# SAIC-MONTREAL/multimodal-dynamics

Measured on AMD Instinct MI355X. Metric: visuotactile samples/sec (train) + ELBO vs CPU ref, cnn-mvae 64x64 bs256 @1/2/4/8 GPU, higher is better.
Workload: dtype f32x3; 1 GPU; cnn-mvae visuotactile+pose 64x64, bs=256 per GPU, fp32 storage and results, GEMMs in the fp32x3 arithmetic (exact three-term bf16 split of the fp32 operands, six of nine products on the bf16 matrix cores, fp32 accumulate; error vs fp64 <= native fp32 MFMA), seq_modeling train step (7 subset ELBOs + backward + Adam), BASELINE configs[1]; global_batch=256, parallelism=dp1, bn=local, launch=hip_graph

## Files before the change

include/mmdyn_hip.h:

```cpp
#ifndef MMDYN_HIP_H
#define MMDYN_HIP_H

#include <stdint.h>

#ifdef __cplusplus
extern "C" {
#endif

#define MMDYN_OK 0
#define MMDYN_ERR_SHAPE (-1)
#define MMDYN_ERR_NULL (-2)
#define MMDYN_ERR_RANGE (-3)

#define MMDYN_ACT_NONE 0
#define MMDYN_ACT_SWISH 1
#define MMDYN_ACT_RELU 2

#define MMDYN_DENSE 0
#define MMDYN_CONV 1
#define MMDYN_TCONV_S2P1 2
#define MMDYN_IM2COL3 3

#define MMDYN_TCONV_S1P0 4

// ... 333 lines not shown
                      int Wi, int Cg, int stride, int offset, int chunks, int flags, void* stream);
int mmdyn_split_planes(const float* x, void* planes, int64_t rows, int C, void* stream);
int mmdyn_igemm_planes_served(int mode, int G, int Bg, int Hi, int Wi, int Cin, int Ho, int Wo, int N);
int mmdyn_bn_swish_fwd_planes(const float* y, const float* mean, const float* rstd, const float* gamma, const float* beta,
                              float* a, void* a_planes, int G, int rows_per_group, int C, void* stream);
int mmdyn_bn_swish_bwd_apply_planes(const float* da, const float* y, const float* mean, const float* rstd, const float* gamma,
                                    const float* beta, const float* sums, float* dy, void* dy_planes, int G, int rows_per_group,
                                    int C, int da_is_du, void* stream);
int mmdyn_conv3_fwd_planes(const float* x, const float* Wp, float* C, void* act_planes, int G, int Bg, int H, int act,
                           void* stream);
int mmdyn_conv3_dgrad_bn_stats(const float* dlogits, const float* Wp, float* stats, const float* y, const float* mean,
                               const float* rstd, const float* gamma, const float* beta, int G, int Bg, int H, void* stream);
int mmdyn_conv3_dgrad_bn_apply_planes(const float* dlogits, const float* Wp, const float* y, const float* mean,
                                      const float* rstd, const float* gamma, const float* beta, const float* sums,
                                      void* dy_planes, int G, int Bg, int H, void* stream);
int mmdyn_bn_eval_swish_bwd(const float* da, const float* y, const float* mean, const float* rstd, const float* gamma,
                            const float* beta, float* dy, void* dy_planes, float* partial, int G, int rows_per_group, int C,
                            int da_is_du, void* stream);
int mmdyn_bn_swish_fwd_b16(const uint16_t* y, const float* mean, const float* rstd, const float* gamma,
                           const float* beta, uint16_t* a, int G, int rows_per_group, int C, int half, void* stream);
int mmdyn_bn_swish_bwd_reduce_b16(const uint16_t* da, const uint16_t* y, const float* mean, const float* rstd,
                                  const float* gamma, const float* beta, float* partial, int G, int rows_per_group,
                                  int C, int half, void* stream);
int mmdyn_bn_swish_bwd_apply_b16(const uint16_t* da, const uint16_t* y, const float* mean, const float* rstd,
                                 const float* gamma, const float* beta, const float* sums, uint16_t* dy, int G,
                                 int rows_per_group, int C, int da_is_du, int half, void* stream);
int mmdyn_act_bwd_b16(const uint16_t* dh, const uint16_t* u, uint16_t* du, int64_t n, int act, int half, void* stream);
int mmdyn_tconv_out3_fwd_b16(const uint16_t* a, const float* w, float* out, int Bt, int Hi, int Wi, int half,
                             void* stream);

// ... 13 lines not shown
```

multimodal-dynamics_amd/csrc/bn.hip:

```cpp
#include "common.h"

namespace {

static int tile_rows_for(int rows_per_group) {
  int t = rows_per_group / 256 / 32 * 32;
  return t < 32 ? 32 : (t > 512 ? 512 : t);
}

struct BnParams {
  const float* mean;
  const float* rstd;
  const float* gamma;
  const float* beta;
};

template <int MODE, typename TA>
__global__ __launch_bounds__(256) void colreduce_kernel(const TA* __restrict__ y,
                                                        const TA* __restrict__ da, BnParams bp,
                                                        float* __restrict__ partial, int rows_per_group,
                                                        int C, int T, int tile_rows) {
  __shared__ float red[256 * 8];
  const int tid = threadIdx.x;
  const int g = blockIdx.y, t = blockIdx.x;
  const int CV = C >> 2;
// ... 301 lines not shown
  for (int64_t i = blockIdx.x * (int64_t)blockDim.x + threadIdx.x; i < total8; i += (int64_t)gridDim.x * blockDim.x) {
    const int cv = (int)(i % CV);
    const int64_t row = i / CV;
    const int g = (int)(row / rows_per_group);
    f32x4 v[2], o[2];
    ldv_nt<float>(y + i * 8, v);
    ldv_nt<float>(y + i * 8 + 4, v + 1);
#pragma unroll
    for (int q = 0; q < 2; ++q) {
      const int c0 = cv * 8 + q * 4;
      f32x4 m = *reinterpret_cast<const f32x4*>(bp.mean + (size_t)g * C + c0);
      f32x4 r = *reinterpret_cast<const f32x4*>(bp.rstd + (size_t)g * C + c0);
      f32x4 ga = *reinterpret_cast<const f32x4*>(bp.gamma + c0);
      f32x4 be = *reinterpret_cast<const f32x4*>(bp.beta + c0);
#pragma unroll
      for (int k = 0; k < 4; ++k) o[q][k] = swishf_(ga[k] * ((v[q][k] - m[k]) * r[k]) + be[k]);
    }
    if (a) {
      stv_nt<float>(a + i * 8, o);
      stv_nt<float>(a + i * 8 + 4, o + 1);
    }
    store_planes8(ap + row * 3 * (int64_t)C + cv * 8, C, o[0], o[1]);
  }
}

__global__ void bn_swish_bwd_apply_planes_kernel(const float* __restrict__ da, const float* __restrict__ y, BnParams bp,
                                                 const float* __restrict__ sums, float* __restrict__ dy, bf16_t* __restrict__ dyp,
                                                 int64_t total8, int rows_per_group, int C, int da_is_du) {
  const int CV = C / 8;
  const float inv_n = 1.f / (float)rows_per_group;
  for (int64_t i = blockIdx.x * (int64_t)blockDim.x + threadIdx.x; i < total8; i += (int64_t)gridDim.x * blockDim.x) {
// ... 367 lines not shown
```

multimodal-dynamics_amd/csrc/common.h:

```cpp
#pragma once
#include <hip/hip_runtime.h>
#include <stdint.h>
#include <stdlib.h>
#include "mmdyn_hip.h"

typedef float f32x16 __attribute__((ext_vector_type(16)));
typedef float f32x4 __attribute__((ext_vector_type(4)));

typedef uint16_t bf16_t;
template <typename T> __device__ __forceinline__ f32x4 ld4(const T* p);
template <> __device__ __forceinline__ f32x4 ld4<float>(const float* p) { return *reinterpret_cast<const f32x4*>(p); }
template <> __device__ __forceinline__ f32x4 ld4<bf16_t>(const bf16_t* p) {
  const uint2 u = *reinterpret_cast<const uint2*>(p);
  f32x4 v;
  v[0] = __uint_as_float(u.x << 16);
  v[1] = __uint_as_float(u.x & 0xffff0000u);
  v[2] = __uint_as_float(u.y << 16);
  v[3] = __uint_as_float(u.y & 0xffff0000u);
  return v;
}
template <typename T> __device__ __forceinline__ float ld1(const T* p);
template <> __device__ __forceinline__ float ld1<float>(const float* p) { return *p; }
template <> __device__ __forceinline__ float ld1<bf16_t>(const bf16_t* p) { return __uint_as_float((uint32_t)*p << 16); }
__device__ __forceinline__ uint32_t pack2_bf16(float lo, float hi) {
// ... 232 lines not shown
  v = wave_sum_d(v);
  __shared__ double red[4];
  if ((threadIdx.x & 63) == 0) red[threadIdx.x >> 6] = v;
  __syncthreads();
  if (threadIdx.x == 0) atomicAdd(dst, scale * (red[0] + red[1] + red[2] + red[3]));
}

constexpr float POE_EPS = 1e-8f;

constexpr uint32_t ALL_PRESENT = 0x01010101u;
__device__ __forceinline__ bool has(uint32_t word, int m) { return ((word >> (8 * m)) & 0xffu) != 0u; }

__device__ __forceinline__ float sigmoid_exact(float v) { return 1.f / (1.f + expf(-v)); }
__device__ __forceinline__ float sigmoidf_(float x) { return __builtin_amdgcn_rcpf(1.0f + __expf(-x)); }
__device__ __forceinline__ float swishf_(float x) { return x * sigmoidf_(x); }
__device__ __forceinline__ float swish_gradf_(float x) {
  float s = sigmoidf_(x);
  return s * (1.0f + x * (1.0f - s));
}
__device__ __forceinline__ float bn_swish_bwd_dy(float du, float xh, float ga, float r, float s0, float s1, float inv_n,
                                                 bool tail_fused) {
#pragma clang fp contract(off)
  const float t0 = __builtin_fmaf(-inv_n, s0, du);
  const float s1n = inv_n * s1;
  const float t = tail_fused ? __builtin_fmaf(-s1n, xh, t0) : t0 - s1n * xh;
  return (ga * r) * t;
}
__device__ __forceinline__ float apply_act(float x, int act) {
  if (act == MMDYN_ACT_SWISH) return swishf_(x);
  if (act == MMDYN_ACT_RELU) return x > 0.f ? x : 0.f;
// ... 45 lines not shown
```

multimodal-dynamics_amd/csrc/tconv_patch.hip:

```cpp
#include "igemm_geom.h"

namespace {

struct PatchEpi {
  const float* bias;
  float* C_act;
  int act;
  const float* bn_y;
  const float* bn_mean;
  const float* bn_rstd;
  const float* bn_gamma;
  const float* bn_beta;
  int bwd_act;
};

typedef __bf16 bf16x8v __attribute__((ext_vector_type(8)));

template <int H, int W, int CIN, int N, int TH, bool P3>
struct PatchCfg {
  static constexpr int CP = CIN + 4, PW2 = W + 2, PH2 = TH + 2;
  static constexpr int ROWB = P3 ? 6 * CIN : 4 * CIN;
  static constexpr int PSB = P3 ? 6 * CIN + 32 : 4 * CP;
  static constexpr int PPP = ROWB / 16;
  static constexpr int NT = N / 16, MT = TH * W / 16 / 8;
  static constexpr int TILES = H / TH;
  static constexpr int SLICE_V = N * PPP;
  static constexpr int NWL = (SLICE_V + 511) / 512;
  static constexpr size_t SMEM = (size_t)(PH2 * PW2 + 2 * N) * PSB;
  static_assert(H % TH == 0 && (TH * W) % 128 == 0 && (W & (W - 1)) == 0 && W >= 16 && CIN % 32 == 0 && N % 16 == 0, "tile geometry");
  static_assert(!P3 || (PSB / 32) % 2 == 1, "plane rows: a stride of 32 * odd bytes");
  static_assert(SMEM <= 160 * 1024, "LDS of one CU");
};

template <int H, int W, int CIN, int N, int TH, bool P3, bool BWD>
__global__ __launch_bounds__(512) void tconv_patch_kernel(const void* __restrict__ X, const void* __restrict__ Wp,
                                                          float* __restrict__ Y, float* __restrict__ stats, int Bt, int Bg,
                                                          int ldc, const PatchEpi ep) {
  using K = PatchCfg<H, W, CIN, N, TH, P3>;
  constexpr int PW2 = K::PW2, PH2 = K::PH2, NT = K::NT, MT = K::MT, PSB = K::PSB, PPP = K::PPP, ROWB = K::ROWB, NWL = K::NWL;
  extern __shared__ __attribute__((aligned(16))) char smem[];
  char* patch = smem;
  char* Bs = smem + PH2 * PW2 * PSB;
  const char* Xb = static_cast<const char*>(X);
  const char* Wb = static_cast<const char*>(Wp);
  const int tid = threadIdx.x, lane = tid & 63, wave = tid >> 6;
  const int r = lane & 15, q = lane >> 4;
  auto widx = [](int s) {
    const int ph = s >> 3, pw = (s >> 2) & 1, th = (s >> 1) & 1, tw = s & 1;
    return (1 - ph + 2 * th) * 4 + (1 - pw + 2 * tw);
  };
  constexpr int RD = 4;
  u32x4_t rb[RD][NWL];
  auto bload = [&](int s, u32x4_t (&dst)[NWL]) {
#pragma unroll
// ... 4 lines not shown
  };
  auto bstore = [&](int slot, const u32x4_t (&src)[NWL]) {
#pragma unroll
    for (int k = 0; k < NWL; ++k) {
      const int i = tid + 512 * k, n = i / PPP, c = i - n * PPP;
      if (i < K::SLICE_V) *reinterpret_cast<u32x4_t*>(Bs + ((size_t)slot * N + n) * PSB + c * 16) = src[k];
    }
  };
  int py_[MT], px_[MT];
#pragma unroll
  for (int m = 0; m < MT; ++m) {
    const int p = (wave * MT + m) * 16 + r;
    py_[m] = p / W;
    px_[m] = p % W;
  }
  constexpr int NPIECE = PH2 * PW2 * PPP, NLD = (NPIECE + 511) / 512;
  const int total = Bt * K::TILES;
  u32x4_t pv[NLD];
  unsigned pok = 0;
  auto pload = [&](int u, int k0, int k1) {
    const int b = u / K::TILES, y0 = (u - b * K::TILES) * TH;
    int t = tid;
    asm volatile("" : "+v"(t));
#pragma unroll
    for (int k = 0; k < NLD; ++k) {
      if (k < k0 || k >= k1) continue;
      const int i = t + 512 * k;
      const int c = i % PPP, p = i / PPP;
      const int py = p / PW2, px = p - py * PW2;
      const int iy = y0 + py - 1, ix = px - 1;
      const bool ok = i < NPIECE && iy >= 0 && iy < H && ix >= 0 && ix < W;
      pok = (pok & ~(1u << k)) | (ok ? 1u << k : 0u);
      pv[k] = __builtin_nontemporal_load(
          reinterpret_cast<const u32x4_t*>(Xb + (ok ? (((size_t)b * H + iy) * W + ix) * ROWB + c * 16 : (size_t)0)));
    }
  };
  auto pstore = [&](int k0, int k1) {
    const u32x4_t z = {0u, 0u, 0u, 0u};
    int t = tid;
    asm volatile("" : "+v"(t));
#pragma unroll
    for (int k = 0; k < NLD; ++k) {
      if (k < k0 || k >= k1) continue;
      const int i = t + 512 * k;
      if (i < NPIECE) *reinterpret_cast<u32x4_t*>(patch + (size_t)(i / PPP) * PSB + (i % PPP) * 16) = ((pok >> k) & 1u) ? pv[k] : z;
    }
  };
  constexpr int NPRE = BWD ? NLD / 2 : NLD, NH = NLD;
  if ((int)blockIdx.x < total) {
    pload(blockIdx.x, 0, NPRE);
#pragma unroll
    for (int k = 0; k < RD; ++k) bload(k, rb[k]);
  }
  for (int u = blockIdx.x; u < total; u += gridDim.x) {
    const int b = u / K::TILES, y0 = (u - b * K::TILES) * TH;
    pload(u, NPRE, NH);
    __syncthreads();
    pstore(0, NH);
    bstore(0, rb[0]);
    __syncthreads();
    if (u + (int)gridDim.x < total) pload(u + gridDim.x, 0, NPRE);
    float colsum[NT], colsq[NT];
#pragma unroll
    for (int n = 0; n < NT; ++n) colsum[n] = colsq[n] = 0.f;
    const int grp_b = b / Bg;
    constexpr bool bnbwd = BWD;
    float bn_m[NT], bn_r[NT], bn_g[NT], bn_b[NT], bias_v[NT];
#pragma unroll
    for (int n = 0; n < NT; ++n) {
      const int col = n * 16 + r;
      const bool bn = bnbwd && ep.bn_mean != nullptr;
      bn_m[n] = bn ? ep.bn_mean[(size_t)grp_b * N + col] : 0.f;
      bn_r[n] = bn ? ep.bn_rstd[(size_t)grp_b * N + col] : 1.f;
      bn_g[n] = bn ? ep.bn_gamma[col] : 1.f;
      bn_b[n] = bn ? ep.bn_beta[col] : 0.f;
      bias_v[n] = ep.bias ? ep.bias[col] : 0.f;
// ... 9 lines not shown
      if constexpr (bnbwd) {
#pragma unroll
        for (int m = 0; m < MT; ++m)
#pragma unroll
          for (int e = 0; e < 4; ++e) {
            const int p = (wave * MT + m) * 16 + 4 * q + e;
            const int y = y0 + p / W, x = p % W;
            const size_t ooff = ((((size_t)b * 2 * H + (2 * y + ph)) * 2 * W) + (2 * x + pw)) * ldc + r;
#pragma unroll
            for (int n = 0; n < NT; ++n) yv[m][e][n] = ep.bn_y[ooff + n * 16];
          }
      }
#pragma unroll
      for (int tap = 0; tap < 4; ++tap) {
        const int s = cls * 4 + tap, slot = tap & 1;
        if (s + 1 < 16) bstore(slot ^ 1, rb[(tap + 1) % RD]);
        bload((s + RD) & 15, rb[tap % RD]);
        const int dh = ph - (tap >> 1), dw = pw - (tap & 1);
        if constexpr (P3) {
          const char* bbase = Bs + ((size_t)slot * N + r) * PSB + q * 16;
          const char* abase[MT];
#pragma unroll
          for (int m = 0; m < MT; ++m) abase[m] = patch + ((size_t)(py_[m] + dh + 1) * PW2 + (px_[m] + dw + 1)) * PSB + q * 16;
          constexpr int order[6][2] = {{0, 2}, {2, 0}, {1, 1}, {0, 1}, {1, 0}, {0, 0}};
#pragma unroll
          for (int kk = 0; kk < CIN / 32; ++kk) {
            bf16x8v bf[NT][3];
#pragma unroll
            for (int n = 0; n < NT; ++n)
#pragma unroll
// ... 99 lines not shown
  if (Hi == 32 && Cin == 32) return 2;
  if (Hi == 64 && Cin == 32) return 8;
  return 0;
}

template <int H, int W, int CIN, int N, int TH, bool P3>
int patch_launch(const void* A, const void* Bp, float* C, float* stats, const IgemmGeom& g, const PatchEpi& ep, hipStream_t st) {
  using K = PatchCfg<H, W, CIN, N, TH, P3>;
  static LdsOptIn lds_opt_in;
  static LdsOptIn lds_opt_in_bwd;
  const int Bt = g.G * g.Bg;
  const int grid = Bt * K::TILES < device_cus() ? Bt * K::TILES : device_cus();
  if (ep.bn_y) {
    if (int e = lds_opt_in_bwd.ensure((const void*)tconv_patch_kernel<H, W, CIN, N, TH, P3, true>, (int)K::SMEM)) return e;
    hipLaunchKernelGGL((tconv_patch_kernel<H, W, CIN, N, TH, P3, true>), dim3(grid), dim3(512), K::SMEM, st, A, Bp, C, stats, Bt, g.Bg,
                       g.ldc, ep);
  } else {
    if (int e = lds_opt_in.ensure((const void*)tconv_patch_kernel<H, W, CIN, N, TH, P3, false>, (int)K::SMEM)) return e;
    hipLaunchKernelGGL((tconv_patch_kernel<H, W, CIN, N, TH, P3, false>), dim3(grid), dim3(512), K::SMEM, st, A, Bp, C, stats, Bt, g.Bg,
                       g.ldc, ep);
  }
  MMDYN_LAUNCH_CHECK();
}

template <bool P3>
int patch_go(const void* A, const void* Bp, const float* bias, float* C, float* C_act, float* stats, float* ws, const IgemmGeom& g,
             hipStream_t st) {
  if (ws || g.splitk != 1) return MMDYN_ERR_SHAPE;
  if (g.bn_y && g.ldc != g.N) return MMDYN_ERR_SHAPE;
  const PatchEpi ep{bias, C_act, g.act, g.bn_y, g.bn_mean, g.bn_rstd, g.bn_gamma, g.bn_beta, g.bwd_act};
  if (g.Hi == 16) return patch_launch<16, 16, 64, 32, 16, P3>(A, Bp, C, stats, g, ep, st);
  if (g.Hi == 32) return patch_launch<32, 32, 32, 32, 16, P3>(A, Bp, C, stats, g, ep, st);
  return patch_launch<64, 64, 32, 32, 8, P3>(A, Bp, C, stats, g, ep, st);
}

// ... 10 lines not shown
bool mmdyn_tconv_patch_plan(const IgemmGeom& g, bool planes, IgemmPlan* p) {
  if (planes && !(patch_p3_enabled() && g.G > 0 && g.Bg > 0)) return false;
  const int tiles = patch_tiles(g.mode, g.Hi, g.Wi, g.Cin, g.Ho, g.Wo, g.N);
  if (!tiles) return false;
  *p = IgemmPlan{};
  p->family = IGEMM_PATCH;
  p->planes = planes;
  p->stat_tiles = g.Bg * tiles;
  return true;
}

int mmdyn_tconv_patch_launch(const void* A, const void* Bp, const float* bias, float* C, float* C_act, float* stats, float* ws,
                             const IgemmGeom& g, const IgemmPlan& p, hipStream_t st) {
  return p.planes ? patch_go<true>(A, Bp, bias, C, C_act, stats, ws, g, st) : patch_go<false>(A, Bp, bias, C, C_act, stats, ws, g, st);
}
```

multimodal-dynamics_amd/mmdyn_hip/_lib.py:

```python
import ctypes
import os

_HERE = os.path.dirname(os.path.abspath(__file__))
LIB_PATH = os.environ.get("MMDYN_HIP_LIB") or os.path.join(_HERE, "libmmdyn_hip.so")

_P, _I, _L, _F, _Q = ctypes.c_void_p, ctypes.c_int, ctypes.c_int64, ctypes.c_float, ctypes.c_uint64


class PassExperts(ctypes.Structure):
    _fields_ = [("mu", _P * 4), ("lv", _P * 4), ("dmu", _P * 4), ("dlv", _P * 4), ("ld", _I * 4), ("dz", _P * 3),
                ("zdst", _P * 3), ("zpl", _P * 3)]


class PackEntry(ctypes.Structure):
    _fields_ = [("src", _P), ("dst", _P), ("kind", _I), ("rows_in", _I), ("cols_in", _I), ("rows_out", _I),
                ("cols_out", _I), ("ld_out", _I), ("dst_bf16", _I)]


class FeedGroups(ctypes.Structure):
    _fields_ = [("recon", _P * 4), ("obs", _P * 4), ("out", _P * 4), ("row_len", _I * 4), ("logits", _I * 4), ("column", _I * 4)]


class GatherGroups(ctypes.Structure):
    _fields_ = [("src", _P * 4), ("out", _P * 4), ("row_len", _I * 4), ("logits", _I * 4)]
# ... 93 lines not shown
    "mmdyn_grad_clip_coef": "p" + "ff" + "p",
    "mmdyn_adam_step_clipped": "pppppp" + "l" + "fffff" + "i" + "p",
    "mmdyn_sgd_step_clipped": "pppp" + "l" + "ffff" + "i" + "p",
    "mmdyn_ema_tick": "pp" + "p",
    "mmdyn_ema_update": "ppp" + "l" + "p",
    "mmdyn_adam_step_ema": "pppppppp" + "l" + "fffff" + "i" + "p",
    "mmdyn_igemm_nt_mx": "pppppppppppp" + "iiiiiiiiiiiiii" + "i" + "pp",
    "mmdyn_wgrad_tn_mx": "ppp" + "iiiiiiiiiii" + "i" + "p",
    "mmdyn_split_planes": "pp" + "l" + "i" + "p",
    "mmdyn_igemm_planes_served": "iiiiiiiii",
    "mmdyn_bn_swish_fwd_planes": "ppppppp" + "iii" + "p",
    "mmdyn_bn_swish_bwd_apply_planes": "ppppppppp" + "iiii" + "p",
    "mmdyn_conv3_fwd_planes": "pppp" + "iiii" + "p",
    "mmdyn_conv3_dgrad_bn_stats": "pppppppp" + "iii" + "p",
    "mmdyn_conv3_dgrad_bn_apply_planes": "ppppppppp" + "iii" + "p",
    "mmdyn_bn_eval_swish_bwd": "ppppppppp" + "iiii" + "p",
    "mmdyn_bn_swish_fwd_b16": "pppppp" + "iiii" + "p",
    "mmdyn_bn_swish_bwd_reduce_b16": "ppppppp" + "iiii" + "p",
    "mmdyn_bn_swish_bwd_apply_b16": "pppppppp" + "iiiii" + "p",
    "mmdyn_act_bwd_b16": "ppp" + "l" + "ii" + "p",
    "mmdyn_tconv_out3_fwd_b16": "ppp" + "iiii" + "p",
    "mmdyn_resize_ksize": "ii",
    "mmdyn_resize_plan": "ii" + "pp",
    "mmdyn_resize_u8_to_chw_f32": "ppp" + "iiiii" + "pppp" + "p",
    "mmdyn_nchw_to_nhwc": "pp" + "iii" + "p",
    "mmdyn_nhwc_to_nchw": "pp" + "iii" + "p",
    "mmdyn_tconv_out3_bn_bce_rows": "ppppppp" + "i" + "pp" + "i" + "ppp" + "iiiiii" + "p",
    "mmdyn_bce_logits_rows_groups": "ppp" + "i" + "ppp" + "iiiii" + "p",
    "mmdyn_mse_rows_groups": "pppp" + "iiii" + "p",
    "mmdyn_kl_rows": "ppp" + "iii" + "p",
# ... 75 lines not shown
```

multimodal-dynamics_amd/mmdyn_hip/engine.py:

```python
import collections.abc
import math
import numbers
import os
import torch

from . import layers, ops
from .models.shapes import DROPOUT_P

FUSED_BCE = True
COPY_MANY = True

SUBSETS_POSE = [(1, 1, 0), (1, 0, 0), (0, 1, 0), (1, 1, 1), (1, 0, 1), (0, 1, 1), (0, 0, 1)]
SUBSETS_NOPOSE = SUBSETS_POSE[:3]
PRECISIONS = ("fp32", "fp32x3", "bf16", "bf16s", "fp16", "fp16s")


def _select_precision(precision):
    prev = (getattr(ops.B, "precision", "fp32"), getattr(ops.B, "fp32_split", False))
    ops.B.precision = "fp32" if precision == "fp32x3" else precision
    ops.B.fp32_split = precision == "fp32x3"
    return prev


def _restore_precision(prev):
# ... 1372 lines not shown
        else:
            ops.B.poe_fwd_avail([p], [avail], eps, mu, lv, z, None, True, 1, B, L)
        return mu, lv, z

    def _zero_latent(self, B):
        z = self._zeros.get(B)
        if z is None:
            z = self._zeros[B] = torch.zeros(B, self.L, device=self.dev)
        return z

    def _decode(self, z, cond=None):
        LN = self.lanes
        LN.fork()
        with LN.lane(0):
            v, _ = layers.run(layers.decoder_forward_steps(self.P["vd"], self.buf["vd"], z, packed=self.pk["vd"], cond=cond,
                                                           training=False))
        with LN.lane(1):
            t, _ = layers.run(layers.decoder_forward_steps(self.P["td"], self.buf["td"], z, packed=self.pk["td"], cond=cond,
                                                           training=False))
        pr = layers.pose_decoder_forward(self.P["pd"], z)[0] if self.use_pose else None
        LN.join()
        return v, t, pr

    def _sample(self, n, cond=None):
        with self._index_scope():
            return self._decode(self._draw_latent(n), cond)[:2]

    def _draw_latent(self, n):
        z = self.noise.eps((n, self.L), self.dev)
        self.noise.commit()
        return z

    def _run(self, key, fn, new_inputs):
        prev_act, prev_w = layers.ACT_DTYPE, layers.W_DTYPE
# ... 802 lines not shown
```

multimodal-dynamics_amd/mmdyn_hip/layers.py:

```python
import weakref

import torch

from . import ops
from .ops import ACT_NONE, ACT_SWISH, ACT_RELU, DENSE, CONV, TCONV_S2P1, IM2COL3, TCONV_S1P0
from .models.shapes import BN_EPS, BN_MOMENTUM, FEAT


def _new(like, *shape, dtype=torch.float32):
    if isinstance(like, ops.Planes):
        like = like.t
    return torch.empty(shape, device=like.device, dtype=dtype)


ACT_DTYPE = torch.float32
W_DTYPE = torch.float32


def _act(like, *shape):
    return torch.empty(shape, device=like.device, dtype=ACT_DTYPE)


def _cdiv(a, b):
    return (a + b - 1) // b
# ... 41 lines not shown

def _plane_twin(Wp):
    ent = PLANE_TWIN.get(Wp.data_ptr())
    if ent is None:
        return None
    if ent[0]() is not Wp:
        if ent[0]() is None:
            del PLANE_TWIN[Wp.data_ptr()]
        return None
    return ent[1]


PATCH_PLANES = True
CONV1_PLANES = True
OUT3_RECOMPUTE = True
WGRAD_ONCE = True
WGRAD_ONCE_PERMS = (1,)


def _conv3_plane_op(name, switch, S, *tensors):
    if not switch or S != 64 or ACT_DTYPE != torch.float32 or any(t.dtype != torch.float32 for t in tensors):
        return None
    return getattr(ops.B, name, None)


def planes_served(mode, G, Bg, Hi, Cin, Ho, N):
    served = getattr(ops.B, "igemm_planes_served", None) if PLANES else None
    if N == 32 and not PATCH_PLANES:
        return False
    return bool(served is not None and ACT_DTYPE == torch.float32 and served(mode, G, Bg, Hi, Hi, Cin, Ho, Ho, N))


def split_operands(x, Wp, mode, G, Bg, Hi, Cin, Ho, N):
    if isinstance(Wp, ops.Planes):
        return x, Wp
    xin = x.t if isinstance(x, ops.Planes) else x
    if xin.dtype not in (torch.float32, torch.bfloat16) or Wp.dtype != torch.float32 or not planes_served(mode, G, Bg, Hi, Cin, Ho, N):
        if isinstance(x, ops.Planes):
# ... 706 lines not shown
        wgrad(du1, c["x"], grads["conv_net.0.weight"], IM2COL3, Bt, S // 2, 32, S, 64, cg_canon=48)
    if not need_dx:
        return None
    dx = _new(c["x"], Bt, 3, S, S)
    ops.B.tconv_out3_fwd(du1, P["conv_net.0.weight"], dx, Bt, S // 2, S // 2)
    return dx


DEC_KEYS = dec_keys(0)


def decoder_forward(*a, **k):
    return run(decoder_forward_steps(*a, **k))


def decoder_forward_steps(P, buf, z, G=1, repeat=1, logits=True, packed=None, cond=None, training=True, loss=None, z_planes=None):
    Bt, L0 = z.shape
    Bg = Bt // G
    convs, last, S = dec_layout(P)
    pk = packed if packed is not None else pack_now(decoder_pack_specs(P))
    Lc = P["upsample.0.weight"].shape[1]
    L = _pad32(Lc)
    if cond is not None or L != L0:
        z = concat_condition(z, cond, L, Lc - L0)
    c = {"Bt": Bt, "G": G, "Bg": Bg, "L": L, "L0": L0, "Lc": Lc, "z": z, "pk": pk, "S": S, "last": last,
         "training": bool(training)}
    c0 = P[f"hallucinate.{convs[0]}.weight"].shape[0]
    want0 = planes_served(TCONV_S1P0, G, Bg, 5, c0, 8, P[f"hallucinate.{convs[0]}.weight"].shape[1])
    fc_planes = (want0 and z_planes is not None and cond is None and L == L0 and ACT_DTYPE == torch.float32
                 and FEAT % c0 == 0 and dense_planes_served(Bt, L, FEAT) and _plane_twin(pk["Wu"]) is not None)
    if fc_planes:
        u0, h0 = dense(z, pk["Wu"], pk["bu"], Bt, L, FEAT, ACT_SWISH, want_act=True, A_planes=z_planes, act_planes=c0)
    else:
        u0, h0 = dense(z, pk["Wu"], pk["bu"], Bt, L, FEAT, ACT_SWISH, want_act=True,
                       act_dtype=ACT_DTYPE if ACT_DTYPE != torch.float32 else None)
    yield
    stages, a, H = [], h0, 5
    if want0 and not fc_planes:
        a = as_planes(h0, c0)
    for j, i in enumerate(convs):
        cin, cout = P[f"hallucinate.{i}.weight"].shape[0], P[f"hallucinate.{i}.weight"].shape[1]
        bn = _bn_of(P, buf, f"hallucinate.{i + 1}")
        if j == 0:
            Ho = H + 3
            y, st, T = tconv_s1p0(a, pk["W1s"], G, Bg, cin, cout, stats=training)
        else:
            Ho = 2 * H
            y, st, T = conv_like(a, pk[f"W{j + 1}s"], TCONV_S2P1, G, Bg, H, cin, Ho, cout, stats=training)
        if j == len(convs) - 1 and fuses_last_bn(S) and cout == 32:
            m, r = bn_stats_only(y, st, T, bn, G, Bg * Ho * Ho, cout, repeat)
            an = None
        else:
            want = j + 1 < len(convs) and planes_served(TCONV_S2P1, G, Bg, Ho, cout, 2 * Ho,
                                                                     P[f"hallucinate.{convs[j + 1]}.weight"].shape[1])
            an, m, r = bn_swish_from_partials(y, st, T, bn, G, Bg * Ho * Ho, cout, repeat, planes=want)
        stages.append(dict(i=i, Hi=H, Ho=Ho, cin=cin, cout=cout, a_in=a, y=y, a=an, m=m, r=r, bn=bn))
        a, H = an, Ho
        yield
    out = None
    c["loss_fused"] = False
    if logits:
        t = stages[-1]
        if t["a"] is None and loss is not None:
            keep = loss.get("keep")
            out = _new(z, Bt if keep is None else Bg, 3, S, S)
            bn_args = (t["y"], t["m"], t["r"], t["bn"].gamma, t["bn"].beta, P[f"hallucinate.{last}.weight"], out,
                       -1 if keep is None else keep, loss["target"])
            mk = dict(mask=loss.get("mask"), mask_channels=loss.get("mask_channels", 1))
            if loss.get("rows") is not None and loss.get("weights") is not None and loss["want_grad"]:
                c["dl"] = _new(z, Bt, 3, S, S)
# ... 184 lines not shown
```

multimodal-dynamics_amd/mmdyn_hip/ops.py:

```python
import ctypes
import numbers

import os

import torch

from . import _lib
from ._lib import PassExperts, FeedGroups, GatherGroups, EnsembleGroups, QuantileGroups, MAX_PASSES, MAX_EXPERTS, FEED_GROUPS, check

ACT_NONE, ACT_SWISH, ACT_RELU = 0, 1, 2
DENSE, CONV, TCONV_S2P1, IM2COL3, TCONV_S1P0 = 0, 1, 2, 3, 4
ROW_GROUPS_MAX = 8
PLAN_TOP_MAX = 8
REFIT_N_MAX = 4096
QUANTILES_MAX = 8
QUANTILE_N_MAX = 128


def _ptr(t, dtype=torch.float32):
    if t is None:
        return None
    if not t.is_cuda:
        raise RuntimeError("mmdyn_hip: the HIP path needs GPU tensors (got a CPU tensor); there is no CPU fallback")
    if t.dtype != dtype:
# ... 464 lines not shown
        check(self.lib.mmdyn_col2im_k4(_ptr(col), _ptr(out), Bt, Hi, Wi, Ho, Wo, C, ldcol, stride, pad,
                                       int(tap_major), _stream()), "mmdyn_col2im_k4")

    def tconv_out3_fwd(self, a, w, out, Bt, Hi, Wi):
        pa, a16 = _aptr(a)
        if a16:
            check(self.lib.mmdyn_tconv_out3_fwd_b16(pa, _ptr(w), _ptr(out), Bt, Hi, Wi, _half(a16), _stream()),
                  "mmdyn_tconv_out3_fwd_b16")
            return
        check(self.lib.mmdyn_tconv_out3_fwd(pa, _ptr(w), _ptr(out), Bt, Hi, Wi, _stream()), "mmdyn_tconv_out3_fwd")

    def tconv_out3_bn_fwd(self, y, mean, rstd, gamma, beta, w, out, G, Bg, Hi, Wi):
        py, y16 = _aptr(y)
        check(self.lib.mmdyn_tconv_out3_bn_fwd(py, _ptr(mean), _ptr(rstd), _ptr(gamma), _ptr(beta), _ptr(w), _ptr(out), G, Bg, Hi, Wi,
                                               y16, _stream()), "mmdyn_tconv_out3_bn_fwd")

    def tconv_out3_bn_bce(self, y, mean, rstd, gamma, beta, w, logits, logits_group, target, dlogit, loss_slots, slot_of_group,
                          grad_scale, G, Bg, Hi, Wi, mask=None, mask_channels=1, unmasked_slots=None):
        py, y16 = _aptr(y)
        if len(slot_of_group) != G or tuple(target.shape) != (Bg, 3, 2 * Hi, 2 * Wi):
            raise ValueError("mmdyn_hip: tconv_out3_bn_bce: one slot per group and a [Bg][3][2Hi][2Wi] target")
        if logits is not None and logits.numel() != (G if logits_group < 0 else 1) * Bg * 3 * 4 * Hi * Wi:
            raise ValueError("mmdyn_hip: tconv_out3_bn_bce: logits buffer of the wrong size")
        if dlogit is not None and dlogit.numel() != G * Bg * 3 * 4 * Hi * Wi:
            raise ValueError("mmdyn_hip: tconv_out3_bn_bce: dlogit buffer of the wrong size")
        if mask is not None and tuple(mask.shape) != (Bg, mask_channels, 2 * Hi, 2 * Wi):
            raise ValueError(f"mmdyn_hip: tconv_out3_bn_bce: mask {tuple(mask.shape)} is not [Bg][{mask_channels}][2Hi][2Wi]")
        slots = (ctypes.c_int * G)(*[int(s) for s in slot_of_group])
        check(self.lib.mmdyn_tconv_out3_bn_bce(py, _ptr(mean), _ptr(rstd), _ptr(gamma), _ptr(beta), _ptr(w), _ptr(logits),
                                               int(logits_group), _ptr(target), _ptr(mask), int(mask_channels), _ptr(dlogit),
# ... 1013 lines not shown
```

multimodal-dynamics_amd/mmdyn_hip/profiling.py:

```python
import collections

import torch

from . import ops

PAD_CYCLES = 100000
HOST_ONLY = {"igemm_stat_tiles", "colstats_tiles", "wgrad_chunks", "igemm_planes_served", "wgrad_canon_served"}


def _canon(name, a):
    if name == "igemm_nt_dgrad_bn":
        A, Bp, C, stats, y, mean, rstd, gamma, beta, mode, G, Bg, Hi, Wi, Cin, Ho, Wo, N, stride, offset = a
        name, a = "igemm_nt", (A, Bp, y, C, None, stats, None, mode, G, Bg, Hi, Wi, Cin, Ho, Wo, N, N, stride, offset, 0, 1)
    if name == "igemm_nt_dgrad_act":
        A, Bp, C, u, act, mode, G, Bg, Hi, Wi, Cin, Ho, Wo, N, stride, offset = a
        name, a = "igemm_nt", (A, Bp, u, C, None, None, None, mode, G, Bg, Hi, Wi, Cin, Ho, Wo, N, N, stride, offset, 0, 1)
    if name == "igemm_nt_grouped":
        A, Bp, bias, C, C_act, u, G, rows, K, N, act = a
        name, a = "igemm_nt", (A, Bp, bias if u is None else u, C, C_act, None, None, ops.DENSE, G, rows, 1, 1, K, 1, 1, N, N, 1, 0, act, 1)
    if name == "wgrad_tn_grouped":
        D, Gt, partial, G, rows, Cd, Cg, chunks = a
        name, a = "wgrad_tn", (D, Gt, partial, ops.DENSE, G * rows, 1, 1, Cd, 1, 1, Cg, 1, 0, chunks)
    if name == "wgrad_tn_canon":
        D, Gt, canon, G, rows, Cd, Cg, cg_canon, perm, beta, chunks = a
        name, a = "wgrad_tn", (D, Gt, canon, ops.DENSE, G * rows, 1, 1, Cd, 1, 1, Cg, 1, 0, chunks)
    if name == "wgrad_out3_bn":
        y, mean, rstd, gamma, beta, Gt, partial, G, Bg, Hr, chunks = a
        return "conv3_wgrad", (y, Gt, partial, ops.IM2COL3, G * Bg, Hr, Hr, 32, 2 * Hr, 2 * Hr, 64, 1, 0, chunks)
    if name == "tconv_out3_bn_fwd":
        return "tconv_out3_fwd", a
    if name == "conv3_fwd_planes":
        x, Wp, C, planes, G, Bg, H, act = a
        return "conv3_nt", (x, Wp, None, C, planes, None, None, ops.IM2COL3, G, Bg, H, H, 64, H // 2, H // 2, 32, 32, 1, 0, act, 1)
    if name == "conv3_dgrad_bn_stats":
        x, Wp, stats, y, mean, rstd, gamma, beta, G, Bg, H = a
        return "conv3_nt", (x, Wp, y, None, None, stats, None, ops.IM2COL3, G, Bg, H, H, 64, H // 2, H // 2, 32, 32, 1, 0, 0, 1)
    if name == "conv3_dgrad_bn_apply_planes":
        x, Wp, y, mean, rstd, gamma, beta, sums, planes, G, Bg, H = a
        return "conv3_nt", (x, Wp, y, planes, None, None, None, ops.IM2COL3, G, Bg, H, H, 64, H // 2, H // 2, 32, 32, 1, 0, 0, 1)
    if name == "igemm_nt" and a[7] == ops.IM2COL3 and a[10] in (64, 128, 256) and \
            tuple(a[10:17]) == (a[10], a[10], 64, a[10] // 2, a[10] // 2, 32, 32):
        return "conv3_nt", a
    if name == "igemm_nt" and a[7] == ops.TCONV_S2P1 and tuple(a[10:16]) in ((16, 16, 64, 32, 32, 32), (32, 32, 32, 64, 64, 32),
                                                                            (64, 64, 32, 128, 128, 32)) and \
            getattr(ops.B, "precision", "fp32") == "fp32" and all(not torch.is_tensor(t) or t.dtype == torch.float32 for t in a[:4]):
# ... 110 lines not shown
```

Before: 55350 samples/s.

## Fuse BN+swish and bf16 plane split into the 16x16 tconv patch kernel prologue

Adds an IBN variant of the tconv patch kernel that loads the raw fp32 pre-BN activations and applies batch-norm plus swish in registers. It splits the result into three bf16 planes while staging the patch into LDS, and optionally writes those planes to global memory for backward. The decoder's 16x16x64 -> 32x32x32 stage now calls this fused op after computing stats only, which skips the separate bn_swish_fwd_planes pass and its read and write of the activation. Eval decoders skip the plane write. BN math is interleaved into the MFMA tap loop, which raises register pressure and adds ALU work inside the kernel.

```diff
diff --git a/include/mmdyn_hip.h b/include/mmdyn_hip.h
--- a/include/mmdyn_hip.h
+++ b/include/mmdyn_hip.h
@@ -371,6 +371,8 @@
 int mmdyn_conv3_dgrad_bn_apply_planes(const float* dlogits, const float* Wp, const float* y, const float* mean,
                                       const float* rstd, const float* gamma, const float* beta, const float* sums,
                                       void* dy_planes, int G, int Bg, int H, void* stream);
+int mmdyn_tconv_patch_bn_fwd(const float* y, const float* mean, const float* rstd, const float* gamma, const float* beta,
+                             const void* w_planes, float* out, float* stats, void* act_planes, int G, int Bg, int Hi, void* stream);
 int mmdyn_bn_eval_swish_bwd(const float* da, const float* y, const float* mean, const float* rstd, const float* gamma,
                             const float* beta, float* dy, void* dy_planes, float* partial, int G, int rows_per_group, int C,
                             int da_is_du, void* stream);
diff --git a/multimodal-dynamics_amd/csrc/bn.hip b/multimodal-dynamics_amd/csrc/bn.hip
--- a/multimodal-dynamics_amd/csrc/bn.hip
+++ b/multimodal-dynamics_amd/csrc/bn.hip
@@ -339,7 +339,7 @@
       f32x4 ga = *reinterpret_cast<const f32x4*>(bp.gamma + c0);
       f32x4 be = *reinterpret_cast<const f32x4*>(bp.beta + c0);
 #pragma unroll
-      for (int k = 0; k < 4; ++k) o[q][k] = swishf_(ga[k] * ((v[q][k] - m[k]) * r[k]) + be[k]);
+      for (int k = 0; k < 4; ++k) o[q][k] = bn_swish_fwd_elem(v[q][k], m[k], r[k], ga[k], be[k]);
     }
     if (a) {
       stv_nt<float>(a + i * 8, o);
diff --git a/multimodal-dynamics_amd/csrc/common.h b/multimodal-dynamics_amd/csrc/common.h
--- a/multimodal-dynamics_amd/csrc/common.h
+++ b/multimodal-dynamics_amd/csrc/common.h
@@ -270,6 +270,11 @@
 __device__ __forceinline__ float sigmoid_exact(float v) { return 1.f / (1.f + expf(-v)); }
 __device__ __forceinline__ float sigmoidf_(float x) { return __builtin_amdgcn_rcpf(1.0f + __expf(-x)); }
 __device__ __forceinline__ float swishf_(float x) { return x * sigmoidf_(x); }
+__device__ __forceinline__ float bn_swish_fwd_elem(float y, float m, float r, float ga, float be) {
+#pragma clang fp contract(off)
+  const float xh = (y - m) * r;
+  return swishf_(__builtin_fmaf(ga, xh, be));
+}
 __device__ __forceinline__ float swish_gradf_(float x) {
   float s = sigmoidf_(x);
   return s * (1.0f + x * (1.0f - s));
diff --git a/multimodal-dynamics_amd/csrc/tconv_patch.hip b/multimodal-dynamics_amd/csrc/tconv_patch.hip
--- a/multimodal-dynamics_amd/csrc/tconv_patch.hip
+++ b/multimodal-dynamics_amd/csrc/tconv_patch.hip
@@ -14,7 +14,16 @@
   int bwd_act;
 };
 
+struct PatchIn {
+  const float* mean;
+  const float* rstd;
+  const float* gamma;
+  const float* beta;
+  bf16_t* planes;
+};
+
 typedef __bf16 bf16x8v __attribute__((ext_vector_type(8)));
+typedef unsigned u32x2_t __attribute__((ext_vector_type(2)));
 
 template <int H, int W, int CIN, int N, int TH, bool P3>
 struct PatchCfg {
@@ -32,12 +41,14 @@
   static_assert(SMEM <= 160 * 1024, "LDS of one CU");
 };
 
-template <int H, int W, int CIN, int N, int TH, bool P3, bool BWD>
+template <int H, int W, int CIN, int N, int TH, bool P3, bool BWD, bool IBN = false>
 __global__ __launch_bounds__(512) void tconv_patch_kernel(const void* __restrict__ X, const void* __restrict__ Wp,
                                                           float* __restrict__ Y, float* __restrict__ stats, int Bt, int Bg,
-                                                          int ldc, const PatchEpi ep) {
+                                                          int ldc, const PatchEpi ep, const PatchIn in) {
   using K = PatchCfg<H, W, CIN, N, TH, P3>;
+  static_assert(!IBN || (P3 && !BWD && K::TILES == 1 && CIN % 4 == 0 && 512 % (CIN / 4) == 0), "IBN: the plane forward, one tile per image");
   constexpr int PW2 = K::PW2, PH2 = K::PH2, NT = K::NT, MT = K::MT, PSB = K::PSB, PPP = K::PPP, ROWB = K::ROWB, NWL = K::NWL;
+  constexpr int XROWB = IBN ? 4 * CIN : ROWB, XPPP = XROWB / 16;
   extern __shared__ __attribute__((aligned(16))) char smem[];
   char* patch = smem;
   char* Bs = smem + PH2 * PW2 * PSB;
@@ -72,7 +83,7 @@
     py_[m] = p / W;
     px_[m] = p % W;
   }
-  constexpr int NPIECE = PH2 * PW2 * PPP, NLD = (NPIECE + 511) / 512;
+  constexpr int NPIECE = PH2 * PW2 * XPPP, NLD = (NPIECE + 511) / 512;
   const int total = Bt * K::TILES;
   u32x4_t pv[NLD];
   unsigned pok = 0;
@@ -84,16 +95,16 @@
     for (int k = 0; k < NLD; ++k) {
       if (k < k0 || k >= k1) continue;
       const int i = t + 512 * k;
-      const int c = i % PPP, p = i / PPP;
+      const int c = i % XPPP, p = i / XPPP;
       const int py = p / PW2, px = p - py * PW2;
       const int iy = y0 + py - 1, ix = px - 1;
       const bool ok = i < NPIECE && iy >= 0 && iy < H && ix >= 0 && ix < W;
       pok = (pok & ~(1u << k)) | (ok ? 1u << k : 0u);
       pv[k] = __builtin_nontemporal_load(
-          reinterpret_cast<const u32x4_t*>(Xb + (ok ? (((size_t)b * H + iy) * W + ix) * ROWB + c * 16 : (size_t)0)));
-    }
-  };
-  auto pstore = [&](int k0, int k1) {
+          reinterpret_cast<const u32x4_t*>(Xb + (ok ? (((size_t)b * H + iy) * W + ix) * XROWB + c * 16 : (size_t)0)));
+    }
+  };
+  auto pstore = [&](int u, int k0, int k1) {
     const u32x4_t z = {0u, 0u, 0u, 0u};
     int t = tid;
     asm volatile("" : "+v"(t));
@@ -101,23 +112,74 @@
     for (int k = 0; k < NLD; ++k) {
       if (k < k0 || k >= k1) continue;
       const int i = t + 512 * k;
-      if (i < NPIECE) *reinterpret_cast<u32x4_t*>(patch + (size_t)(i / PPP) * PSB + (i % PPP) * 16) = ((pok >> k) & 1u) ? pv[k] : z;
+      if constexpr (IBN) {
+        if (i < NPIECE) {
+          const int c = i % XPPP, p = i / XPPP;
+          const bool ok = (pok >> k) & 1u;
+          const f32x4 a = __builtin_bit_cast(f32x4, pv[k]);
+          uint32_t h0, h1, m0, m1, l0, l1;
+          split3_bf16(a[0], a[1], h0, m0, l0);
+          split3_bf16(a[2], a[3], h1, m1, l1);
+          const u32x2_t z2 = {0u, 0u};
+          const u32x2_t hi = ok ? u32x2_t{h0, h1} : z2, mid = ok ? u32x2_t{m0, m1} : z2, lo = ok ? u32x2_t{l0, l1} : z2;
+          char* dst = patch + (size_t)p * PSB + c * 8;
+          *reinterpret_cast<u32x2_t*>(dst) = hi;
+          *reinterpret_cast<u32x2_t*>(dst + 2 * CIN) = mid;
+          *reinterpret_cast<u32x2_t*>(dst + 4 * CIN) = lo;
+          if (in.planes != nullptr && ok) {
+            const int py = p / PW2, px = p - py * PW2;
+            char* g = reinterpret_cast<char*>(in.planes) + (((size_t)u * H + (py - 1)) * W + (px - 1)) * (6 * CIN) + c * 8;
+            __builtin_nontemporal_store(hi, reinterpret_cast<u32x2_t*>(g));
+            __builtin_nontemporal_store(mid, reinterpret_cast<u32x2_t*>(g + 2 * CIN));
+            __builtin_nontemporal_store(lo, reinterpret_cast<u32x2_t*>(g + 4 * CIN));
+          }
+        }
+      } else {
+        if (i < NPIECE) *reinterpret_cast<u32x4_t*>(patch + (size_t)(i / PPP) * PSB + (i % PPP) * 16) = ((pok >> k) & 1u) ? pv[k] : z;
+      }
+    }
+  };
+  f32x4 in_m = {0.f, 0.f, 0.f, 0.f}, in_r = in_m, in_g = in_m, in_b = in_m;
+  const int c4 = IBN ? (tid % XPPP) * 4 : 0;
+  if constexpr (IBN) {
+    in_g = *reinterpret_cast<const f32x4*>(in.gamma + c4);
+    in_b = *reinterpret_cast<const f32x4*>(in.beta + c4);
+  }
+  auto ppar = [&](int u) {
+    const int grp = (u / K::TILES) / Bg;
+    in_m = *reinterpret_cast<const f32x4*>(in.mean + (size_t)grp * CIN + c4);
+    in_r = *reinterpret_cast<const f32x4*>(in.rstd + (size_t)grp * CIN + c4);
+  };
+  auto pact = [&](int k0, int k1) {
+#pragma unroll
+    for (int k = 0; k < NLD; ++k) {
+      if (k < k0 || k >= k1) continue;
+      f32x4 v = __builtin_bit_cast(f32x4, pv[k]);
+#pragma unroll
+      for (int e = 0; e < 4; ++e) v[e] = bn_swish_fwd_elem(v[e], in_m[e], in_r[e], in_g[e], in_b[e]);
+      pv[k] = __builtin_bit_cast(u32x4_t, v);
     }
   };
   constexpr int NPRE = BWD ? NLD / 2 : NLD, NH = NLD;
   if ((int)blockIdx.x < total) {
+    if constexpr (IBN) ppar(blockIdx.x);
     pload(blockIdx.x, 0, NPRE);
 #pragma unroll
     for (int k = 0; k < RD; ++k) bload(k, rb[k]);
+    if constexpr (IBN) pact(0, NLD);
   }
   for (int u = blockIdx.x; u < total; u += gridDim.x) {
     const int b = u / K::TILES, y0 = (u - b * K::TILES) * TH;
     pload(u, NPRE, NH);
     __syncthreads();
-    pstore(0, NH);
+    pstore(u, 0, NH);
     bstore(0, rb[0]);
     __syncthreads();
-    if (u + (int)gridDim.x < total) pload(u + gridDim.x, 0, NPRE);
+    const bool more = u + (int)gridDim.x < total;
+    if constexpr (IBN) {
+      if (more) ppar(u + gridDim.x);
+    }
+    if (more) pload(u + gridDim.x, 0, NPRE);
     float colsum[NT], colsq[NT];
 #pragma unroll
     for (int n = 0; n < NT; ++n) colsum[n] = colsq[n] = 0.f;
@@ -157,6 +219,10 @@
 #pragma unroll
       for (int tap = 0; tap < 4; ++tap) {
         const int s = cls * 4 + tap, slot = tap & 1;
+        if constexpr (IBN) {
+          if (more && cls == 1) pact(2 * tap, 2 * tap + 2);
+          if (more && cls == 2) pact(8 + tap, 9 + tap);
+        }
         if (s + 1 < 16) bstore(slot ^ 1, rb[(tap + 1) % RD]);
         bload((s + RD) & 15, rb[tap % RD]);
         const int dh = ph - (tap >> 1), dw = pw - (tap & 1);
@@ -286,11 +352,11 @@
   if (ep.bn_y) {
     if (int e = lds_opt_in_bwd.ensure((const void*)tconv_patch_kernel<H, W, CIN, N, TH, P3, true>, (int)K::SMEM)) return e;
     hipLaunchKernelGGL((tconv_patch_kernel<H, W, CIN, N, TH, P3, true>), dim3(grid), dim3(512), K::SMEM, st, A, Bp, C, stats, Bt, g.Bg,
-                       g.ldc, ep);
+                       g.ldc, ep, PatchIn{});
   } else {
     if (int e = lds_opt_in.ensure((const void*)tconv_patch_kernel<H, W, CIN, N, TH, P3, false>, (int)K::SMEM)) return e;
     hipLaunchKernelGGL((tconv_patch_kernel<H, W, CIN, N, TH, P3, false>), dim3(grid), dim3(512), K::SMEM, st, A, Bp, C, stats, Bt, g.Bg,
-                       g.ldc, ep);
+                       g.ldc, ep, PatchIn{});
   }
   MMDYN_LAUNCH_CHECK();
 }
@@ -331,3 +397,21 @@
                              const IgemmGeom& g, const IgemmPlan& p, hipStream_t st) {
   return p.planes ? patch_go<true>(A, Bp, bias, C, C_act, stats, ws, g, st) : patch_go<false>(A, Bp, bias, C, C_act, stats, ws, g, st);
 }
+
+extern "C" int mmdyn_tconv_patch_bn_fwd(const float* y, const float* mean, const float* rstd, const float* gamma, const float* beta,
+                                        const void* w_planes, float* out, float* stats, void* act_planes, int G, int Bg, int Hi,
+                                        void* stream) {
+  if (!y || !mean || !rstd || !gamma || !beta || !w_planes || !out) return MMDYN_ERR_NULL;
+  if (G <= 0 || Bg <= 0 || Hi != 16 || !patch_enabled() || !patch_p3_enabled()) return MMDYN_ERR_SHAPE;
+  const int64_t Bt = (int64_t)G * Bg;
+  if (Bt * 16 * 16 * 64 >= (1LL << 31) || Bt * 32 * 32 * 32 >= (1LL << 31)) return MMDYN_ERR_RANGE;
+  using K = PatchCfg<16, 16, 64, 32, 16, true>;
+  static LdsOptIn lds_opt_in;
+  const auto kernel = tconv_patch_kernel<16, 16, 64, 32, 16, true, false, true>;
+  if (int e = lds_opt_in.ensure((const void*)kernel, (int)K::SMEM)) return e;
+  const int grid = Bt < device_cus() ? (int)Bt : device_cus();
+  const PatchIn in{mean, rstd, gamma, beta, static_cast<bf16_t*>(act_planes)};
+  hipLaunchKernelGGL(kernel, dim3(grid), dim3(512), K::SMEM, (hipStream_t)stream, (const void*)y, w_planes, out, stats, (int)Bt, Bg,
+                     32, PatchEpi{}, in);
+  MMDYN_LAUNCH_CHECK();
+}
diff --git a/multimodal-dynamics_amd/mmdyn_hip/_lib.py b/multimodal-dynamics_amd/mmdyn_hip/_lib.py
--- a/multimodal-dynamics_amd/mmdyn_hip/_lib.py
+++ b/multimodal-dynamics_amd/mmdyn_hip/_lib.py
@@ -131,6 +131,7 @@
     "mmdyn_conv3_fwd_planes": "pppp" + "iiii" + "p",
     "mmdyn_conv3_dgrad_bn_stats": "pppppppp" + "iii" + "p",
     "mmdyn_conv3_dgrad_bn_apply_planes": "ppppppppp" + "iii" + "p",
+    "mmdyn_tconv_patch_bn_fwd": "ppppppppp" + "iii" + "p",
     "mmdyn_bn_eval_swish_bwd": "ppppppppp" + "iiii" + "p",
     "mmdyn_bn_swish_fwd_b16": "pppppp" + "iiii" + "p",
     "mmdyn_bn_swish_bwd_reduce_b16": "ppppppp" + "iiii" + "p",
diff --git a/multimodal-dynamics_amd/mmdyn_hip/engine.py b/multimodal-dynamics_amd/mmdyn_hip/engine.py
--- a/multimodal-dynamics_amd/mmdyn_hip/engine.py
+++ b/multimodal-dynamics_amd/mmdyn_hip/engine.py
@@ -1410,10 +1410,10 @@
         LN.fork()
         with LN.lane(0):
             v, _ = layers.run(layers.decoder_forward_steps(self.P["vd"], self.buf["vd"], z, packed=self.pk["vd"], cond=cond,
-                                                           training=False))
+                                                           training=False, backward=False))
         with LN.lane(1):
             t, _ = layers.run(layers.decoder_forward_steps(self.P["td"], self.buf["td"], z, packed=self.pk["td"], cond=cond,
-                                                           training=False))
+                                                           training=False, backward=False))
         pr = layers.pose_decoder_forward(self.P["pd"], z)[0] if self.use_pose else None
         LN.join()
         return v, t, pr
diff --git a/multimodal-dynamics_amd/mmdyn_hip/layers.py b/multimodal-dynamics_amd/mmdyn_hip/layers.py
--- a/multimodal-dynamics_amd/mmdyn_hip/layers.py
+++ b/multimodal-dynamics_amd/mmdyn_hip/layers.py
@@ -79,6 +79,7 @@
 PATCH_PLANES = True
 CONV1_PLANES = True
 OUT3_RECOMPUTE = True
+PATCH_BN = True
 WGRAD_ONCE = True
 WGRAD_ONCE_PERMS = (1,)
 
@@ -87,6 +88,17 @@
     if not switch or S != 64 or ACT_DTYPE != torch.float32 or any(t.dtype != torch.float32 for t in tensors):
         return None
     return getattr(ops.B, name, None)
+
+
+def _patch_bn_op(Wp, G, Bg, Hi, Cin, N, *tensors):
+    if not PATCH_BN or ACT_DTYPE != torch.float32 or any(t.dtype != torch.float32 for t in tensors):
+        return None
+    if (Hi, Cin, N) != (16, 64, 32) or not planes_served(TCONV_S2P1, G, Bg, Hi, Cin, 2 * Hi, N):
+        return None
+    wp = _plane_twin(Wp)
+    if wp is None or wp.C != Cin or wp.rows * Cin != Wp.numel():
+        return None
+    return getattr(ops.B, "tconv_patch_bn_fwd", None)
 
 
 def planes_served(mode, G, Bg, Hi, Cin, Ho, N):
@@ -823,7 +835,8 @@
     return run(decoder_forward_steps(*a, **k))
 
 
-def decoder_forward_steps(P, buf, z, G=1, repeat=1, logits=True, packed=None, cond=None, training=True, loss=None, z_planes=None):
+def decoder_forward_steps(P, buf, z, G=1, repeat=1, logits=True, packed=None, cond=None, training=True, loss=None, z_planes=None,
+                          backward=True):
     Bt, L0 = z.shape
     Bg = Bt // G
     convs, last, S = dec_layout(P)
@@ -847,12 +860,22 @@
     stages, a, H = [], h0, 5
     if want0 and not fc_planes:
         a = as_planes(h0, c0)
+    patch_bn = None
     for j, i in enumerate(convs):
         cin, cout = P[f"hallucinate.{i}.weight"].shape[0], P[f"hallucinate.{i}.weight"].shape[1]
         bn = _bn_of(P, buf, f"hallucinate.{i + 1}")
         if j == 0:
             Ho = H + 3
             y, st, T = tconv_s1p0(a, pk["W1s"], G, Bg, cin, cout, stats=training)
+        elif patch_bn is not None:
+            Ho, t = 2 * H, stages[-1]
+            y, st, T = _new(z, Bt * Ho * Ho, cout), None, 0
+            if training:
+                T = ops.B.igemm_stat_tiles(TCONV_S2P1, G, Bg, H, H, cin, Ho, Ho, cout, planes=True)
+                st = _new(z, G, T, 2, cout)
+            a = ops.Planes(Bt * H * H, cin, z.device) if backward else None
+            patch_bn(t["y"], t["m"], t["r"], t["bn"].gamma, t["bn"].beta, _plane_twin(pk[f"W{j + 1}s"]), y, st, a, G, Bg, H)
+            t["a"] = a
         else:
             Ho = 2 * H
             y, st, T = conv_like(a, pk[f"W{j + 1}s"], TCONV_S2P1, G, Bg, H, cin, Ho, cout, stats=training)
@@ -862,7 +885,13 @@
         else:
             want = j + 1 < len(convs) and planes_served(TCONV_S2P1, G, Bg, Ho, cout, 2 * Ho,
                                                                      P[f"hallucinate.{convs[j + 1]}.weight"].shape[1])
-            an, m, r = bn_swish_from_partials(y, st, T, bn, G, Bg * Ho * Ho, cout, repeat, planes=want)
+            patch_bn = None
+            if want:
+                patch_bn = _patch_bn_op(pk[f"W{j + 2}s"], G, Bg, Ho, cout, P[f"hallucinate.{convs[j + 1]}.weight"].shape[1], y)
+            if patch_bn is not None:
+                (m, r), an = bn_stats_only(y, st, T, bn, G, Bg * Ho * Ho, cout, repeat), None
+            else:
+                an, m, r = bn_swish_from_partials(y, st, T, bn, G, Bg * Ho * Ho, cout, repeat, planes=want)
         stages.append(dict(i=i, Hi=H, Ho=Ho, cin=cin, cout=cout, a_in=a, y=y, a=an, m=m, r=r, bn=bn))
         a, H = an, Ho
         yield
diff --git a/multimodal-dynamics_amd/mmdyn_hip/ops.py b/multimodal-dynamics_amd/mmdyn_hip/ops.py
--- a/multimodal-dynamics_amd/mmdyn_hip/ops.py
+++ b/multimodal-dynamics_amd/mmdyn_hip/ops.py
@@ -502,6 +502,27 @@
         py, y16 = _aptr(y)
         check(self.lib.mmdyn_tconv_out3_bn_fwd(py, _ptr(mean), _ptr(rstd), _ptr(gamma), _ptr(beta), _ptr(w), _ptr(out), G, Bg, Hi, Wi,
                                                y16, _stream()), "mmdyn_tconv_out3_bn_fwd")
+
+    def tconv_patch_bn_fwd(self, y, mean, rstd, gamma, beta, w_planes, out, stats, act_planes, G, Bg, Hi):
+        if not self._x3():
+            raise ValueError("mmdyn_hip: tconv_patch_bn_fwd belongs to the fp32x3 arithmetic (engine precision 'fp32x3')")
+        Bt = G * Bg
+        if not isinstance(w_planes, Planes) or w_planes.C != 64 or w_planes.rows != 16 * 32 or not w_planes.t.is_cuda \
+                or not w_planes.t.is_contiguous():
+            raise ValueError("mmdyn_hip: tconv_patch_bn_fwd: w_planes must be the [16*32][3][64] plane twin of the packed weight")
+        if y.numel() != Bt * Hi * Hi * 64 or out.numel() != Bt * 4 * Hi * Hi * 32 or mean.numel() != G * 64 or rstd.numel() != G * 64 \
+                or gamma.numel() != 64 or beta.numel() != 64:
+            raise ValueError("mmdyn_hip: tconv_patch_bn_fwd: tensor sizes do not match G, Bg, Hi")
+        if stats is not None and tuple(stats.shape) != (G, Bg, 2, 32):
+            raise ValueError(f"mmdyn_hip: tconv_patch_bn_fwd: stats must be [G={G}][Bg={Bg}][2][32], got {tuple(stats.shape)}")
+        pap = None
+        if act_planes is not None:
+            if not isinstance(act_planes, Planes) or act_planes.rows != Bt * Hi * Hi or act_planes.C != 64 \
+                    or not act_planes.t.is_cuda or not act_planes.t.is_contiguous():
+                raise ValueError("mmdyn_hip: tconv_patch_bn_fwd: act_planes must be a contiguous Planes of [G*Bg*Hi*Hi] rows of 64 channels")
+            pap = act_planes.t.data_ptr()
+        check(self.lib.mmdyn_tconv_patch_bn_fwd(_ptr(y), _ptr(mean), _ptr(rstd), _ptr(gamma), _ptr(beta), w_planes.t.data_ptr(),
+                                                _ptr(out), _ptr(stats), pap, G, Bg, Hi, _stream()), "mmdyn_tconv_patch_bn_fwd")
 
     def tconv_out3_bn_bce(self, y, mean, rstd, gamma, beta, w, logits, logits_group, target, dlogit, loss_slots, slot_of_group,
                           grad_scale, G, Bg, Hi, Wi, mask=None, mask_channels=1, unmasked_slots=None):
diff --git a/multimodal-dynamics_amd/mmdyn_hip/profiling.py b/multimodal-dynamics_amd/mmdyn_hip/profiling.py
--- a/multimodal-dynamics_amd/mmdyn_hip/profiling.py
+++ b/multimodal-dynamics_amd/mmdyn_hip/profiling.py
@@ -29,6 +29,9 @@
         return "conv3_wgrad", (y, Gt, partial, ops.IM2COL3, G * Bg, Hr, Hr, 32, 2 * Hr, 2 * Hr, 64, 1, 0, chunks)
     if name == "tconv_out3_bn_fwd":
         return "tconv_out3_fwd", a
+    if name == "tconv_patch_bn_fwd":
+        y, mean, rstd, gamma, beta, wp, out, stats, planes, G, Bg, Hi = a
+        return "tconv_patch", (y, wp, None, out, planes, stats, None, ops.TCONV_S2P1, G, Bg, Hi, Hi, 64, 2 * Hi, 2 * Hi, 32, 32, 1, 0, 0, 1)
     if name == "conv3_fwd_planes":
         x, Wp, C, planes, G, Bg, H, act = a
         return "conv3_nt", (x, Wp, None, C, planes, None, None, ops.IM2COL3, G, Bg, H, H, 64, H // 2, H // 2, 32, 32, 1, 0, act, 1)
```

Measured after the change: 55730 samples/s, median of 6. Within noise of the previous version (+0.7%).
